# martinambrus/PitchExtractor

Measured on AMD Instinct MI355X. Metric: mel-frames/sec training throughput (JDCNet, 24 kHz, batch=256), higher is better.
Workload: dtype f32

## Files before the change

### pitchextractor_amd/csrc/act16.h

```cpp
#pragma once
#include "common.h"

namespace pe {

typedef __bf16 act16_t;

__device__ __forceinline__ float4 ld4(const float* p) { return *reinterpret_cast<const float4*>(p); }
__device__ __forceinline__ void st4(float* p, const float4& v) { *reinterpret_cast<float4*>(p) = v; }
__device__ __forceinline__ float ld1(const float* p) { return *p; }
__device__ __forceinline__ void st1(float* p, float v) { *p = v; }

__device__ __forceinline__ float4 ld4(const act16_t* p) {
  const uint2 u = *reinterpret_cast<const uint2*>(p);
  return make_float4(__uint_as_float(u.x << 16), __uint_as_float(u.x & 0xffff0000u), __uint_as_float(u.y << 16),
                     __uint_as_float(u.y & 0xffff0000u));
}
__device__ __forceinline__ unsigned pack_bf16_rne(float a, float b) {
  typedef __bf16 b2 __attribute__((ext_vector_type(2)));
  typedef float f2 __attribute__((ext_vector_type(2)));
  const f2 v = {a, b};
  return __builtin_bit_cast(unsigned, __builtin_convertvector(v, b2));
}
__device__ __forceinline__ void st4(act16_t* p, const float4& v) {
  *reinterpret_cast<uint2*>(p) = make_uint2(pack_bf16_rne(v.x, v.y), pack_bf16_rne(v.z, v.w));
}
__device__ __forceinline__ float ld1(const act16_t* p) {
  return __uint_as_float((unsigned)*reinterpret_cast<const unsigned short*>(p) << 16);
}
__device__ __forceinline__ void st1(act16_t* p, float v) { *p = (act16_t)v; }

template <class T> struct RawQuad;
template <> struct RawQuad<float> { typedef float4 type; };
template <> struct RawQuad<act16_t> { typedef uint2 type; };
__device__ __forceinline__ float4 ldraw(const float* p) { return *reinterpret_cast<const float4*>(p); }
__device__ __forceinline__ uint2 ldraw(const act16_t* p) { return *reinterpret_cast<const uint2*>(p); }
__device__ __forceinline__ float4 widen(const float4& v) { return v; }
__device__ __forceinline__ float4 widen(const uint2& u) {
  return make_float4(__uint_as_float(u.x << 16), __uint_as_float(u.x & 0xffff0000u), __uint_as_float(u.y << 16),
                     __uint_as_float(u.y & 0xffff0000u));
}
template <class T> __device__ __forceinline__ typename RawQuad<T>::type ldraw_buffer(__amdgpu_buffer_rsrc_t rs, unsigned voff, unsigned soff);
template <> __device__ __forceinline__ float4 ldraw_buffer<float>(__amdgpu_buffer_rsrc_t rs, unsigned voff, unsigned soff) {
  typedef unsigned int u4 __attribute__((ext_vector_type(4)));
  const u4 d = __builtin_amdgcn_raw_buffer_load_b128(rs, voff, soff, 0);
  return make_float4(__uint_as_float(d.x), __uint_as_float(d.y), __uint_as_float(d.z), __uint_as_float(d.w));
}
template <> __device__ __forceinline__ uint2 ldraw_buffer<act16_t>(__amdgpu_buffer_rsrc_t rs, unsigned voff, unsigned soff) {
  typedef unsigned int u2 __attribute__((ext_vector_type(2)));
  const u2 d = __builtin_amdgcn_raw_buffer_load_b64(rs, voff, soff, 0);
  return make_uint2(d.x, d.y);
}
template <class R> __device__ __forceinline__ R zero_raw();
template <> __device__ __forceinline__ float4 zero_raw<float4>() { return make_float4(0.f, 0.f, 0.f, 0.f); }
template <> __device__ __forceinline__ uint2 zero_raw<uint2>() { return make_uint2(0u, 0u); }

}
```

### pitchextractor_amd/csrc/common.h

```cpp
#pragma once
#include <hip/hip_runtime.h>
#include <stdint.h>
#include "../../include/pitchextractor_hip.h"

#define PE_CHECK_HIP(expr)                              \
  do {                                                  \
    hipError_t _e = (expr);                             \
    if (_e != hipSuccess) return (int)_e;               \
  } while (0)

#define PE_LAUNCH_CHECK()                               \
  do {                                                  \
    hipError_t _e = hipGetLastError();                  \
    if (_e != hipSuccess) return (int)_e;               \
  } while (0)

static inline hipStream_t pe_stream(void* s) { return reinterpret_cast<hipStream_t>(s); }

static inline int pe_unserved(int products) {
  return products >= PE_PROD_NATIVE && products <= PE_PROD_F16 ? PE_E_UNSUPPORTED : PE_E_ARG;
}

static inline int pe_cdiv(long a, long b) { return (int)((a + b - 1) / b); }

typedef float f32x4 __attribute__((ext_vector_type(4)));
typedef float f32x16 __attribute__((ext_vector_type(16)));

#define PE_WAVE 64

__device__ __forceinline__ double pe_wave_strided_sum(const double* base, long stride, int n) {
  const int lane = threadIdx.x & 63;
  double s = 0.0;
  for (int z = lane; z < n; z += 64) s += base[(long)z * stride];
#pragma unroll
  for (int off = 32; off > 0; off >>= 1) s += __shfl_down(s, off, 64);
  return s;
}

static inline int pe_pick_splits(int tiles, long K, int min_k_per_split, int resident) {
  long max_s = K / min_k_per_split;
  if (max_s < 1) max_s = 1;
  if (max_s > 1024) max_s = 1024;
  int best = 1;
  double best_score = -1.0;
  for (int sp = 1; sp <= (int)max_s; ++sp) {
    const long wgs = (long)tiles * sp;
    const long waves = (wgs + resident - 1) / resident;
    const double eff = (double)wgs / (double)(waves * resident);
    const double score = eff - 0.0001 * sp + (wgs >= 2L * resident ? 0.05 : 0.0);
    if (score > best_score) { best_score = score; best = sp; }
  }
  return best;
}

__device__ __forceinline__ float4 pe_ordered_slab_sum4(const float* __restrict__ ws, long slab_stride, int splits,
                                                       long i4) {
  const float4* p = reinterpret_cast<const float4*>(ws) + i4;
  const long st4 = slab_stride >> 2;
  double sx = 0.0, sy = 0.0, sz = 0.0, sw = 0.0;
  int z = 0;
  for (; z + 8 <= splits; z += 8) {
    float4 v[8];
#pragma unroll
    for (int u = 0; u < 8; ++u) v[u] = p[(long)(z + u) * st4];
#pragma unroll
    for (int u = 0; u < 8; ++u) { sx += (double)v[u].x; sy += (double)v[u].y; sz += (double)v[u].z; sw += (double)v[u].w; }
  }
  for (; z < splits; ++z) {
    const float4 v = p[(long)z * st4];
    sx += (double)v.x; sy += (double)v.y; sz += (double)v.z; sw += (double)v.w;
  }
  return make_float4((float)sx, (float)sy, (float)sz, (float)sw);
}

__device__ __forceinline__ void philox_round(uint32_t (&c)[4], uint32_t (&k)[2]) {
  const uint32_t M0 = 0xD2511F53u, M1 = 0xCD9E8D57u;
  const uint64_t p0 = (uint64_t)M0 * c[0], p1 = (uint64_t)M1 * c[2];
  const uint32_t n0 = (uint32_t)(p1 >> 32) ^ c[1] ^ k[0];
  const uint32_t n1 = (uint32_t)p1;
  const uint32_t n2 = (uint32_t)(p0 >> 32) ^ c[3] ^ k[1];
  const uint32_t n3 = (uint32_t)p0;
  c[0] = n0; c[1] = n1; c[2] = n2; c[3] = n3;
  k[0] += 0x9E3779B9u; k[1] += 0xBB67AE85u;
}

__device__ __forceinline__ void philox4(uint64_t seed, uint64_t ctr, uint32_t (&out)[4]) {
  uint32_t c[4] = {(uint32_t)ctr, (uint32_t)(ctr >> 32), 0u, 0u};
  uint32_t k[2] = {(uint32_t)seed, (uint32_t)(seed >> 32)};
#pragma unroll
  for (int i = 0; i < 10; ++i) philox_round(c, k);
  out[0] = c[0]; out[1] = c[1]; out[2] = c[2]; out[3] = c[3];
}

__device__ __forceinline__ bool pe_dropout_keep(uint32_t word, float p) {
  return ((float)(word >> 8) * (1.0f / 16777216.0f)) >= p;
}
```

### pitchextractor_amd/csrc/conv.hip

```cpp
#include <type_traits>
#include "forms.h"

namespace {
using namespace pe;
typedef unsigned int u32x4_t __attribute__((ext_vector_type(4)));
typedef unsigned int u32x2_t __attribute__((ext_vector_type(2)));

__global__ void repack3x3_kernel(const float* __restrict__ w, float* __restrict__ w_fwd,
                                 float* __restrict__ w_dgrad, int Cout, int Cin) {
  const int idx = blockIdx.x * blockDim.x + threadIdx.x;
  if (idx >= Cout * Cin * 9) return;
  const int tap = idx % 9, ci = (idx / 9) % Cin, co = idx / (9 * Cin);
  const float v = w[idx];
  if (w_fwd) w_fwd[((long)co * 9 + tap) * Cin + ci] = v;
  if (w_dgrad) w_dgrad[((long)ci * 9 + (8 - tap)) * Cout + co] = v;
}

__global__ void transpose2d_kernel(const float* __restrict__ in, float* __restrict__ out, int rows, int cols) {
  __shared__ float tile[32][33];
  const int c0 = blockIdx.x * 32, r0 = blockIdx.y * 32;
  for (int i = threadIdx.y; i < 32; i += 8) {
    const int r = r0 + i, c = c0 + threadIdx.x;
    tile[i][threadIdx.x] = (r < rows && c < cols) ? in[(long)r * cols + c] : 0.f;
  }
  __syncthreads();
  for (int i = threadIdx.y; i < 32; i += 8) {
    const int c = c0 + i, r = r0 + threadIdx.x;
    if (r < rows && c < cols) out[(long)c * rows + r] = tile[threadIdx.x][i];
  }
}

template <class TO>
struct ConvEpiT {
  TO* Y;
  int rows, N, accumulate;
  double* stats;
  __device__ __forceinline__ void operator()(int row, int col, float v) const {
    if (row < rows && col < N) {
      TO* d = Y + (long)row * N + col;
      if (accumulate) v += ld1(d);
      st1(d, v);
    }
  }
};
typedef ConvEpiT<float> ConvEpi;

template <class TO> __device__ __forceinline__ float stored_value(float v) {
  if constexpr (std::is_same<TO, float>::value) return v;
  else return __uint_as_float(pack_bf16_rne(v, 0.f) << 16);
}

template <class TL, int MODE, class TA = float, class TH = __bf16>
__global__ __launch_bounds__(256) void conv3x3_kernel(ConvLoader<TL::A_LOADS, TA> al, RowLoader bl, ConvEpiT<TA> ep,
                                                      int K, int tiles_m, int tiles_n, const unsigned* amax_x,
                                                      const unsigned* amax_w) {
  __shared__ __attribute__((aligned(16))) float As[TL::BM * nt_row_floats<MODE>()];
  __shared__ __attribute__((aligned(16))) float Bs[TL::BN * nt_row_floats<MODE>()];
  const int tile = xcd_remap(blockIdx.x, tiles_m * tiles_n);
  const int m0 = (tile / tiles_n) * TL::BM, n0 = (tile % tiles_n) * TL::BN;
  al.init(m0);
  bl.init(n0);
  f32x16 acc[TL::TM][TL::TN];
  zero_acc<TL>(acc);
  H2Scales hs{1.f, 1.f, 1.f};
  if constexpr (MODE == kSplit2) hs.load(amax_x, amax_w);
  nt_mainloop_mode<TL, MODE, false, 1, TH>(al, bl, K, As, Bs, acc, hs.sa, hs.sb);
  for_each_acc<TL>(acc, [&](int r, int c, float v) { ep(m0 + r, n0 + c, MODE == kSplit2 ? hs.unscale(v) : v); });
}

template <class TL, class FM, class TA = typename FM::TA>
int launch_conv(const TA* x, const float* wp, TA* y, int B, int T, int F, int C, int N, int accumulate,
                hipStream_t st, const unsigned* amax_x, const unsigned* amax_w) {
  const int rows = B * T * F, K = 9 * C;
  ConvLoader<TL::A_LOADS, TA> al;
  al.p = x; al.T = T; al.F = F; al.C = C; al.rows = rows;
  RowLoader bl{wp, (long)K, N, K, 0};
  ConvEpiT<TA> ep{y, rows, N, accumulate, nullptr};
  const int tm = pe_cdiv(rows, TL::BM), tn = pe_cdiv(N, TL::BN);
  hipLaunchKernelGGL((conv3x3_kernel<TL, FM::MODE, TA, typename FM::TH>), dim3(tm * tn), dim3(256), 0, st, al, bl, ep, K,
                     tm, tn, amax_x, amax_w);
  PE_LAUNCH_CHECK();
  return PE_OK;
}


template <int NT, class TH = __bf16>
__global__ void wfrag_pack_kernel(const float* __restrict__ w, long ld, int N, int K, uint4* __restrict__ out,
                                  const unsigned* __restrict__ amax = nullptr) {
  const long idx = (long)blockIdx.x * blockDim.x + threadIdx.x;
  const int NB32 = (N + 31) >> 5, KB = K >> 4;
  const int lane = (int)(idx & 63);
  const long blk = idx >> 6;
  if (blk >= (long)NB32 * KB) return;
  const int nb = (int)(blk % NB32), kb = (int)(blk / NB32);
  const int n = nb * 32 + (lane & 31), k = kb * 16 + (lane >> 5) * 8;
  float4 v0 = make_float4(0.f, 0.f, 0.f, 0.f), v1 = v0;
  if (n < N) {
    v0 = *reinterpret_cast<const float4*>(w + (long)n * ld + k);
    v1 = *reinterpret_cast<const float4*>(w + (long)n * ld + k + 4);
  }
  uint4* dst = out + ((long)(kb * NB32 + nb) * NT) * 64 + lane;
  if constexpr (NT == 3) {
    const Split3 a = split3(v0), b = split3(v1);
    dst[0] = make_uint4(a.hi.x, a.hi.y, b.hi.x, b.hi.y);
    dst[64] = make_uint4(a.mid.x, a.mid.y, b.mid.x, b.mid.y);
    dst[128] = make_uint4(a.lo.x, a.lo.y, b.lo.x, b.lo.y);
  } else if constexpr (NT == 2) {
    const float sc = h2_scale(*amax);
    const Split2 a = split2(v0, sc), b = split2(v1, sc);
    dst[0] = make_uint4(a.hi.x, a.hi.y, b.hi.x, b.hi.y);
    dst[64] = make_uint4(a.lo.x, a.lo.y, b.lo.x, b.lo.y);
  } else {
    const half4<TH> a = to_half4<TH>(v0), b = to_half4<TH>(v1);
    const uint2 ua = __builtin_bit_cast(uint2, a), ub = __builtin_bit_cast(uint2, b);
    dst[0] = make_uint4(ua.x, ua.y, ub.x, ub.y);
  }
}

template <int BN, int MODE, int PASSES, int D, bool FA2, class TA = float, class TH = __bf16>
__global__ __launch_bounds__(256, 2) void conv3x3_halo_wf_kernel(const TA* __restrict__ x,
                                                                 const uint4* __restrict__ wf, ConvEpiT<TA> ep, int T,
                                                                 int F, int C, int N, int P, int tiles_m,
                                                                 int tiles_n, const unsigned* amax_x,
                                                                 const unsigned* amax_w) {
  constexpr int NT = mode_terms<MODE>();
  using H = term_t<NT, TH>;
  H2Scales hs{1.f, 1.f, 1.f};
  if constexpr (MODE == kSplit2) hs.load(amax_x, amax_w);
  constexpr int TM = 2, TN = BN / 64, WN = BN / 2;
  constexpr int ZR = PASSES * 32;
  constexpr int AIMG = (ZR + 4) * 32;
  constexpr int S = 18 * TN;
  static_assert(S % D == 0 && D >= 2, "the fragment ring wraps at chunk boundaries");
  __shared__ __attribute__((aligned(16))) H As[NT * AIMG];
  const int tid = threadIdx.x, lane = tid & 63, wv = tid >> 6;
  const int wm = wv >> 1, wn = wv & 1, r = lane & 31, h = lane >> 5;
  const int tile = xcd_remap(blockIdx.x, tiles_m * tiles_n);
  const int p0 = (tile / tiles_n) * 128, n0 = (tile % tiles_n) * BN;
  const int WR = 128 + 2 * F + 2;
  const int srow = tid >> 3, piece = tid & 7;
  const int nchunks = C / 32;

  unsigned vbits[TM];
#pragma unroll
  for (int i = 0; i < TM; ++i) {
    const int p = p0 + wm * 64 + i * 32 + r;
    unsigned b = 0;
    if (p < P) {
      const int f = p % F, t = (p / F) % T;
#pragma unroll
      for (int tap = 0; tap < 9; ++tap) {
        const int tt = t + tap / 3 - 1, ff = f + tap % 3 - 1;
        if (tt >= 0 && tt < T && ff >= 0 && ff < F) b |= 1u << tap;
      }
    }
    vbits[i] = b;
  }

  typedef typename RawQuad<TA>::type Raw;
  Raw ra[PASSES];
  const __amdgpu_buffer_rsrc_t xrs = __builtin_amdgcn_make_buffer_rsrc(
      const_cast<TA*>(x), 0, (unsigned)((long)P * C * (long)sizeof(TA)), 0x00020000);
  unsigned voa[PASSES];
#pragma unroll
  for (int ps = 0; ps < PASSES; ++ps) {
    const int wr = ps * 32 + srow;
    const long q = (long)p0 - F - 1 + wr;
    voa[ps] = (wr < WR && q >= 0 && q < P) ? (unsigned)((q * C + piece * 4) * (long)sizeof(TA)) : 0x80000000u;
  }
  auto fetch_a = [&](int cc) {
    const unsigned so = (unsigned)(cc * 32 * (int)sizeof(TA));
#pragma unroll
    for (int ps = 0; ps < PASSES; ++ps) {
      if constexpr (std::is_same<TA, float>::value) {
        const u32x4_t d = __builtin_amdgcn_raw_buffer_load_b128(xrs, voa[ps], so, 0);
        ra[ps] = make_float4(__uint_as_float(d.x), __uint_as_float(d.y), __uint_as_float(d.z), __uint_as_float(d.w));
      } else {
        const u32x2_t d = __builtin_amdgcn_raw_buffer_load_b64(xrs, voa[ps], so, 0);
        ra[ps] = make_uint2(d.x, d.y);
      }
    }
  };

  const int NB32 = (N + 31) >> 5, kb_tap = C >> 4;
  const int kb_stride = NB32 * NT * 64;
  const __amdgpu_buffer_rsrc_t wrs = __builtin_amdgcn_make_buffer_rsrc(
      const_cast<uint4*>(wf), 0, (unsigned)((long)9 * kb_tap * kb_stride * 16), 0x00020000);
  unsigned vow[TN];
#pragma unroll
  for (int j = 0; j < TN; ++j) {
    const int nb = (n0 + wn * WN + j * 32) >> 5;
    vow[j] = (unsigned)(((nb < NB32 ? nb : NB32 - 1) * NT * 64 + lane) * 16);
  }
  half8<H> ring[D][NT];
  auto issue = [&](int slot, int cc, int s) {
    const int j = s % TN, kk = (s / TN) & 1, tap = s / (2 * TN);
    const unsigned so = (unsigned)((tap * kb_tap + cc * 2 + kk) * kb_stride) * 16u;
#pragma unroll
    for (int c = 0; c < NT; ++c)
      ring[slot][c] = __builtin_bit_cast(half8<H>, __builtin_amdgcn_raw_buffer_load_b128(wrs, vow[j], so + (unsigned)c * 1024u, 0));
  };

  f32x16 acc[TM][TN];
#pragma unroll
  for (int i = 0; i < TM; ++i)
#pragma unroll
    for (int j = 0; j < TN; ++j)
#pragma unroll
      for (int g = 0; g < 16; ++g) acc[i][j][g] = 0.f;

  if (tid < 8) {
#pragma unroll
    for (int c = 0; c < NT; ++c) *reinterpret_cast<uint2*>(As + c * AIMG + ZR * 32 + tid * 4) = make_uint2(0u, 0u);
  }
  fetch_a(0);
#pragma unroll
  for (int s = 0; s < D - 1; ++s) issue(s, 0, s);

  auto load_fa = [&](half8<H> (&fa)[TM][NT], int tap, int kk) {
    const int shift = (tap / 3) * F + tap % 3;
#pragma unroll
    for (int i = 0; i < TM; ++i) {
      const int row = (vbits[i] >> tap) & 1u ? wm * 64 + i * 32 + r + shift : ZR;
#pragma unroll
      for (int c = 0; c < NT; ++c)
        fa[i][c] = *reinterpret_cast<const half8<H>*>(As + c * AIMG + swz_off(row, kk * 2 + h));
    }
  };

  for (int cc = 0; cc < nchunks; ++cc) {
    __syncthreads();
#pragma unroll
    for (int ps = 0; ps < PASSES; ++ps) halo_store<NT>(As, AIMG, ps * 32 + srow, piece, ra[ps], hs.sa);
    __syncthreads();
    if (cc + 1 < nchunks) fetch_a(cc + 1);
    half8<H> fa[FA2 ? 2 : 1][TM][NT];
    if (FA2) load_fa(fa[0], 0, 0);
#pragma unroll
    for (int s = 0; s < S; ++s) {
      const int j = s % TN, blk = s / TN;
      {
        const int sn = s + D - 1;
        if (sn < S) issue(sn % D, cc, sn);
        else if (cc + 1 < nchunks) issue(sn % D, cc + 1, sn - S);
      }
      if (FA2) {
        if (j == 0 && blk + 1 < 18) load_fa(fa[(blk + 1) & 1], (blk + 1) >> 1, (blk + 1) & 1);
      } else if (j == 0) {
        load_fa(fa[0], blk >> 1, blk & 1);
      }
      const int fs = FA2 ? (blk & 1) : 0;
#pragma unroll
      for (int i = 0; i < TM; ++i) acc[i][j] = mfma_terms<NT>(fa[fs][i], ring[s % D], acc[i][j]);
      __builtin_amdgcn_sched_barrier(0);
    }
  }
  double s1[TN], s2[TN];
#pragma unroll
  for (int j = 0; j < TN; ++j) s1[j] = s2[j] = 0.0;
#pragma unroll
  for (int i = 0; i < TM; ++i)
#pragma unroll
    for (int j = 0; j < TN; ++j)
#pragma unroll
      for (int g = 0; g < 16; ++g) {
        const int row = p0 + wm * 64 + i * 32 + (g & 3) + 8 * (g >> 2) + 4 * h, col = n0 + wn * WN + j * 32 + r;
        if (row < ep.rows && col < ep.N) {
          TA* d = ep.Y + (long)row * ep.N + col;
          float v = MODE == kSplit2 ? hs.unscale(acc[i][j][g]) : acc[i][j][g];
          if (ep.accumulate) v += ld1(d);
          st1(d, v);
          v = stored_value<TA>(v);
          s1[j] += (double)v;
          s2[j] += (double)v * (double)v;
        }
      }
  if (ep.stats) {
#pragma unroll
    for (int j = 0; j < TN; ++j) {
      s1[j] += __shfl_xor(s1[j], 32, 64);
      s2[j] += __shfl_xor(s2[j], 32, 64);
    }
    __syncthreads();
    double* red = reinterpret_cast<double*>(As);
    if (h == 0) {
#pragma unroll
      for (int j = 0; j < TN; ++j) {
        red[(wm * BN + wn * WN + j * 32 + r) * 2] = s1[j];
        red[(wm * BN + wn * WN + j * 32 + r) * 2 + 1] = s2[j];
      }
    }
    __syncthreads();
    const long tile_m = tile / tiles_n;
    for (int c = tid; c < BN; c += 256) {
      if (n0 + c < ep.N) {
        ep.stats[(tile_m * 2) * ep.N + n0 + c] = red[c * 2] + red[(BN + c) * 2];
        ep.stats[(tile_m * 2 + 1) * ep.N + n0 + c] = red[c * 2 + 1] + red[(BN + c) * 2 + 1];
      }
    }
  }
}

template <int BN, class FM, int PASSES, int D, bool FA2, class TA = typename FM::TA>
int launch_conv_halo_wf(const TA* x, const void* wf, TA* y, int B, int T, int F, int C, int N, int accumulate,
                        double* stats, hipStream_t st, const unsigned* amax_x, const unsigned* amax_w) {
  const int P = B * T * F;
  ConvEpiT<TA> ep{y, P, N, accumulate, stats};
  const int tm = pe_cdiv(P, 128), tn = pe_cdiv(N, BN);
  hipLaunchKernelGGL((conv3x3_halo_wf_kernel<BN, FM::MODE, PASSES, D, FA2, TA, typename FM::TH>), dim3(tm * tn),
                     dim3(256), 0, st, x, reinterpret_cast<const uint4*>(wf), ep, T, F, C, N, P, tm, tn, amax_x, amax_w);
  PE_LAUNCH_CHECK();
  return PE_OK;
}

static inline size_t pe_wfrag_bytes_host(int N, int K, int terms) { return (size_t)((N + 31) / 32) * (K / 16) * terms * 1024; }

int conv_halo_passes(int F, int N) {
  const int wr = 128 + 2 * F + 2;
  if (wr <= 7 * 32 && N >= 96) return 7;
  if (wr <= 10 * 32 && N <= 64) return 10;
  return 0;
}

template <int BM, int BN>
__global__ __launch_bounds__(256) void conv3x3_wgrad_kernel(const float* __restrict__ dy, const float* __restrict__ x,
                                                            float* __restrict__ ws, int T, int F, int Cin,
                                                            int Cout, int P, int k_per_split, int tiles_n,
                                                            int n_tiles, int n_chunks) {
  __shared__ __attribute__((aligned(16))) float As[kBK * BM];
  __shared__ __attribute__((aligned(16))) float Bs[kBK * BN];
  const int xcd = blockIdx.x & 7, q = blockIdx.x >> 3;
  const int tap = q % 9;
  const int chunk = (q / 9) * 8 + xcd;
  if (chunk >= n_chunks) return;
  const int tile = chunk % n_tiles, split = chunk / n_tiles;
  const int m0 = (tile / tiles_n) * BM, n0 = (tile % tiles_n) * BN;
  const int kb = split * k_per_split;
  const int ke = min(P, kb + k_per_split);
  KRowLoader<BM> al{dy, (long)Cout, Cout, 0};
  ShiftedPixelLoader<BN> bl;
  bl.p = x; bl.T = T; bl.F = F; bl.C = Cin; bl.dt = tap / 3 - 1; bl.df = tap % 3 - 1;
  al.init(m0, kb);
  bl.init(n0, kb);
  f32x16 acc[BM / 64][BN / 64];
#pragma unroll
  for (int i = 0; i < BM / 64; ++i)
#pragma unroll
    for (int j = 0; j < BN / 64; ++j)
#pragma unroll
      for (int g = 0; g < 16; ++g) acc[i][j][g] = 0.f;
  tn_mainloop<BM, BN>(al, bl, kb, ke, As, Bs, acc);
  float* dst = ws + ((long)split * 9 + tap) * Cout * Cin;
  tn_for_each_acc<BM, BN>(acc, [&](int r, int c, float v) {
    const int co = m0 + r, ci = n0 + c;
    if (co < Cout && ci < Cin) dst[(long)co * Cin + ci] = v;
  });
}

template <int DUMMY>
__global__ __launch_bounds__(256, 2) void conv3x3_wgrad9_kernel(const float* __restrict__ dy,
                                                                const float* __restrict__ x,
                                                                float* __restrict__ ws, int T, int F, int Cin,
                                                                int Cout, int P, int k_per_split, int tiles_n) {
  __shared__ __attribute__((aligned(16))) float Ys[kBK * 64];
  __shared__ __attribute__((aligned(16))) float Xs[3 * 34 * 64];
  __shared__ float Mk[3 * 34 * 4];
  const int tid = threadIdx.x, lane = tid & 63, wv = tid >> 6;
  const int wm = wv >> 1, wn = wv & 1, r = lane & 31, h = lane >> 5;
  const int tiles_mn = (Cout / 64) * tiles_n;
  const int lin = xcd_remap(blockIdx.x, gridDim.x);
  const int tile_id = lin % tiles_mn, split_id = lin / tiles_mn;
  const int m0 = (tile_id / tiles_n) * 64, n0 = (tile_id % tiles_n) * 64;
  const int kb = split_id * k_per_split;
  const int ke = min(P, kb + k_per_split);

  f32x16 acc[9];
#pragma unroll
  for (int tp = 0; tp < 9; ++tp)
#pragma unroll
    for (int q = 0; q < 16; ++q) acc[tp][q] = 0.f;

  const int c4 = (tid & 15) * 4;
  float4 ry[2], rx[7];
  auto fetch = [&](int k0) {
#pragma unroll
    for (int i = 0; i < 2; ++i) {
      const int k = k0 + (tid >> 4) + 16 * i;
      ry[i] = k < ke ? *reinterpret_cast<const float4*>(dy + (long)k * Cout + m0 + c4)
                     : make_float4(0.f, 0.f, 0.f, 0.f);
    }
#pragma unroll
    for (int i = 0; i < 7; ++i) {
      const int wr = (tid >> 4) + 16 * i;
      rx[i] = make_float4(0.f, 0.f, 0.f, 0.f);
      if (wr < 102) {
        const int w = wr / 34, row = wr - w * 34;
        const long q = (long)k0 + (long)(w - 1) * F + row - 1;
        if (q >= 0 && q < P) rx[i] = *reinterpret_cast<const float4*>(x + q * Cin + n0 + c4);
      }
    }
  };
  fetch(kb);
  for (int k0 = kb; k0 < ke; k0 += kBK) {
    __syncthreads();
#pragma unroll
    for (int i = 0; i < 2; ++i) *reinterpret_cast<float4*>(Ys + ((tid >> 4) + 16 * i) * 64 + c4) = ry[i];
#pragma unroll
    for (int i = 0; i < 7; ++i) {
      const int wr = (tid >> 4) + 16 * i;
      if (wr < 102) *reinterpret_cast<float4*>(Xs + wr * 64 + c4) = rx[i];
    }
    if (tid < 102) {
      const int w = tid / 34, row = tid - w * 34;
      const long q = (long)k0 + (long)(w - 1) * F + row - 1;
      float m0v = 0.f, m1v = 0.f, m2v = 0.f;
      if (q >= 0 && q < P) {
        const int fq = (int)(q % F), tq = (int)((q / F) % T);
        const bool trow = !((w == 2 && tq == 0) || (w == 0 && tq == T - 1));
        m0v = (trow && fq != F - 1) ? 1.f : 0.f;
        m1v = trow ? 1.f : 0.f;
        m2v = (trow && fq != 0) ? 1.f : 0.f;
      }
      Mk[tid * 4 + 0] = m0v; Mk[tid * 4 + 1] = m1v; Mk[tid * 4 + 2] = m2v;
    }
    __syncthreads();
    if (k0 + kBK < ke) fetch(k0 + kBK);
    const float* a_rd = Ys + wm * 32 + r;
    const float* b_rd = Xs + wn * 32 + r;
#pragma unroll 4
    for (int s = 0; s < kBK / 2; ++s) {
      const int k = 2 * s + h;
      const float a = a_rd[k * 64];
#pragma unroll
      for (int w = 0; w < 3; ++w)
#pragma unroll
        for (int d = 0; d < 3; ++d) {
          const int row = k + d;
          const float b = b_rd[(w * 34 + row) * 64] * Mk[(w * 34 + row) * 4 + d];
          acc[w * 3 + d] = mfma32(a, b, acc[w * 3 + d]);
        }
    }
  }
#pragma unroll
  for (int tp = 0; tp < 9; ++tp) {
    float* dst = ws + ((long)split_id * 9 + tp) * Cout * Cin;
#pragma unroll
    for (int q = 0; q < 16; ++q) {
      const int co = m0 + wm * 32 + (q & 3) + 8 * (q >> 2) + 4 * h;
      const int ci = n0 + wn * 32 + r;
      dst[(long)co * Cin + ci] = acc[tp][q];
    }
  }
}

template <int NT, bool HALO, class TA = float, class TH = __bf16>
__global__ __launch_bounds__(256, 2) void conv3x3_wgrad9_x3_kernel(const TA* __restrict__ dy,
                                                                   const TA* __restrict__ x,
                                                                   float* __restrict__ ws, int T, int F, int Cin,
                                                                   int Cout, int P, int k_per_split, int tiles_n,
                                                                   const unsigned* amax_dy, const unsigned* amax_x) {
// ... 549 lines not shown
```

### pitchextractor_amd/csrc/gemm.hip

```cpp
#include <stdlib.h>
#include <type_traits>
#include <utility>
#include "forms.h"


namespace {
using namespace pe;
typedef unsigned int u32x4 __attribute__((ext_vector_type(4)));

bool aligned16(const void* p) { return (reinterpret_cast<uintptr_t>(p) & 15) == 0; }

template <class TO>
struct StoreEpiT {
  TO* C;
  long ldc;
  const float* bias0;
  const float* bias1;
  int M, N, accumulate;
  __device__ __forceinline__ void operator()(int row, int col, float v) const {
    if (row < M && col < N) {
      if (bias0) v += bias0[col];
      if (bias1) v += bias1[col];
      TO* dst = C + (long)row * ldc + col;
      if (accumulate) v += ld1(dst);
      st1(dst, v);
    }
  }
};
typedef StoreEpiT<float> StoreEpi;

template <class TL, int MODE, class TA = float, class TH = __bf16>
__global__ __launch_bounds__(256) void gemm_nt_kernel(RowLoaderT<TA> al, RowLoader bl, StoreEpiT<TA> ep, int K,
                                                      int tiles_m, int tiles_n, const unsigned* amax_a,
                                                      const unsigned* amax_b) {
  __shared__ __attribute__((aligned(16))) float As[TL::BM * nt_row_floats<MODE>()];
  __shared__ __attribute__((aligned(16))) float Bs[TL::BN * nt_row_floats<MODE>()];
  const int tile = xcd_remap(blockIdx.x, tiles_m * tiles_n);
  const int m0 = (tile / tiles_n) * TL::BM, n0 = (tile % tiles_n) * TL::BN;
  al.init(m0);
  bl.init(n0);
  f32x16 acc[TL::TM][TL::TN];
  zero_acc<TL>(acc);
  H2Scales hs{1.f, 1.f, 1.f};
  if constexpr (MODE == kSplit2) hs.load(amax_a, amax_b);
  nt_mainloop_mode<TL, MODE, false, 1, TH>(al, bl, K, As, Bs, acc, hs.sa, hs.sb);
  for_each_acc<TL>(acc, [&](int r, int c, float v) { ep(m0 + r, n0 + c, MODE == kSplit2 ? hs.unscale(v) : v); });
}

template <class TL, int MODE, class TA = float, class TH = __bf16>
__global__ __launch_bounds__(256, ((MODE == kSplit || MODE == kSplit2) && TL::BM == 128 && TL::BN == 128) ? 3 : 1)
void gemm_nt_t_kernel(RowLoaderT<TA> al, RowLoader bl, StoreEpiT<TA> ep, int K, int tiles_m, int tiles_n,
                      const unsigned* amax_a, const unsigned* amax_b) {
  using TT = Tile<TL::BN, TL::BM, TL::WAVES_N, TL::WAVES_M>;
  __shared__ __attribute__((aligned(16))) float As[TL::BM * nt_row_floats<MODE>()];
  __shared__ __attribute__((aligned(16))) float Bs[TL::BN * nt_row_floats<MODE>()];
  const int tile = xcd_remap(blockIdx.x, tiles_m * tiles_n);
  const int m0 = (tile / tiles_n) * TL::BM, n0 = (tile % tiles_n) * TL::BN;
  al.init(m0);
  bl.init(n0);
  f32x16 acc[TT::TM][TT::TN];
  zero_acc<TT>(acc);
  H2Scales hs{1.f, 1.f, 1.f};
  if constexpr (MODE == kSplit2) hs.load(amax_a, amax_b);
  nt_mainloop_mode<TT, MODE, true, 1, TH>(bl, al, K, Bs, As, acc, hs.sb, hs.sa);
  const int lane = threadIdx.x & 63, wv = threadIdx.x >> 6;
  const int wn = wv / TT::WAVES_N, wm = wv % TT::WAVES_N;
  const int r = lane & 31, h = lane >> 5;
#pragma unroll
  for (int i = 0; i < TT::TM; ++i)
#pragma unroll
    for (int q = 0; q < 4; ++q) {
      const int col = n0 + wn * TT::WM + i * 32 + 8 * q + 4 * h;
      if (col >= ep.N) continue;
      float4 b0 = make_float4(0.f, 0.f, 0.f, 0.f), b1 = b0;
      if (ep.bias0) b0 = make_float4(ep.bias0[col], ep.bias0[col + 1], ep.bias0[col + 2], ep.bias0[col + 3]);
      if (ep.bias1) b1 = make_float4(ep.bias1[col], ep.bias1[col + 1], ep.bias1[col + 2], ep.bias1[col + 3]);
#pragma unroll
      for (int j = 0; j < TT::TN; ++j) {
        const int row = m0 + wm * TT::WN + j * 32 + r;
        if (row >= ep.M) continue;
        TA* dst = ep.C + (long)row * ep.ldc + col;
        float4 v = make_float4(acc[i][j][4 * q], acc[i][j][4 * q + 1], acc[i][j][4 * q + 2], acc[i][j][4 * q + 3]);
        if constexpr (MODE == kSplit2) {
          v.x = hs.unscale(v.x); v.y = hs.unscale(v.y); v.z = hs.unscale(v.z); v.w = hs.unscale(v.w);
        }
        if (ep.bias0) { v.x += b0.x; v.y += b0.y; v.z += b0.z; v.w += b0.w; }
        if (ep.bias1) { v.x += b1.x; v.y += b1.y; v.z += b1.z; v.w += b1.w; }
        if (ep.accumulate) { const float4 o = ld4(dst); v.x += o.x; v.y += o.y; v.z += o.z; v.w += o.w; }
        st4(dst, v);
      }
    }
}

template <class TL, class F, class TA = typename F::TA>
int launch_nt(const RowLoaderT<TA>& al, const RowLoader& bl, const StoreEpiT<TA>& ep, int M, int N, int K,
              hipStream_t st, const unsigned* amax_a, const unsigned* amax_b) {
  constexpr int MODE = F::MODE;
  using TH = typename F::TH;
  const int tm = pe_cdiv(M, TL::BM), tn = pe_cdiv(N, TL::BN);
  const bool vec = MODE != kNative && (N & 3) == 0 && (ep.ldc & 3) == 0 &&
                   (reinterpret_cast<uintptr_t>(ep.C) & (4 * sizeof(TA) - 1)) == 0;
  if (vec)
    hipLaunchKernelGGL((gemm_nt_t_kernel<TL, MODE, TA, TH>), dim3(tm * tn), dim3(256), 0, st, al, bl, ep, K, tm, tn,
                       amax_a, amax_b);
  else
    hipLaunchKernelGGL((gemm_nt_kernel<TL, MODE, TA, TH>), dim3(tm * tn), dim3(256), 0, st, al, bl, ep, K, tm, tn, amax_a,
                       amax_b);
  PE_LAUNCH_CHECK();
  return PE_OK;
}

template <int BM, int BN, int MODE, class TA = float, class TH = __bf16>
__global__ __launch_bounds__(256) void gemm_tn_kernel(KRowLoader<BM, TA> al, KRowLoader<BN, TA> bl, float* out,
                                                      long ldo, long split_stride, int M, int N, int K,
                                                      int k_per_split, int tiles_n, int accumulate,
                                                      const unsigned* amax_a, const unsigned* amax_b) {
  __shared__ __attribute__((aligned(16))) float As[tn_lds_floats<MODE, BM>()];
  __shared__ __attribute__((aligned(16))) float Bs[tn_lds_floats<MODE, BN>()];
  const int tiles_mn = ((M + BM - 1) / BM) * tiles_n;
  const int lin = xcd_remap(blockIdx.x, gridDim.x);
  const int tile_id = lin % tiles_mn, split_id = lin / tiles_mn;
  const int m0 = (tile_id / tiles_n) * BM, n0 = (tile_id % tiles_n) * BN;
  const int kb = split_id * k_per_split;
  const int ke = min(K, kb + k_per_split);
  al.init(m0, kb);
  bl.init(n0, kb);
  f32x16 acc[BM / 64][BN / 64];
#pragma unroll
  for (int i = 0; i < BM / 64; ++i)
#pragma unroll
    for (int j = 0; j < BN / 64; ++j)
#pragma unroll
      for (int g = 0; g < 16; ++g) acc[i][j][g] = 0.f;
  H2Scales hs{1.f, 1.f, 1.f};
  if constexpr (MODE == kSplit2) hs.load(amax_a, amax_b);
  tn_mainloop_mode<MODE, BM, BN, 1, TH>(al, bl, kb, ke, As, Bs, acc, hs.sa, hs.sb);
  float* dst = out + (long)split_id * split_stride;
  tn_for_each_acc<BM, BN>(acc, [&](int r, int c, float v) {
    const int row = m0 + r, col = n0 + c;
    if constexpr (MODE == kSplit2) v = hs.unscale(v);
    if (row < M && col < N) {
      float* d = dst + (long)row * ldo + col;
      if (accumulate) v += *d;
      *d = v;
    }
  });
}

__global__ void splitk_reduce_kernel(const float* ws, long split_stride, int splits, float* C, long ldc,
                                     int M, int N, int accumulate) {
  const long i4 = (long)blockIdx.x * blockDim.x + threadIdx.x;
  if (i4 * 4 >= (long)M * N) return;
  const float4 s = pe_ordered_slab_sum4(ws, split_stride, splits, i4);
  const long idx = i4 * 4;
  const int row = (int)(idx / N), col = (int)(idx - (long)row * N);
  float* d = C + (long)row * ldc + col;
  if (accumulate) { d[0] += s.x; d[1] += s.y; d[2] += s.z; d[3] += s.w; }
  else { d[0] = s.x; d[1] = s.y; d[2] = s.z; d[3] = s.w; }
}

void tn_plan(int M, int N, int K, int bm, int bn, int mode, int* splits, int* k_per_split) {
  const int tiles = pe_cdiv(M, bm) * pe_cdiv(N, bn);
  const int s = pe_pick_splits(tiles, K, 512, (mode == kSplit || mode == kSplit2) ? 512 : 768);
  int kps = pe_cdiv(K, s);
  kps = (kps + kBK - 1) / kBK * kBK;
  *splits = pe_cdiv(K, kps);
  *k_per_split = kps;
}

template <int BM, int BN, class F, class TA = typename F::TA>
int launch_tn(const TA* A, long lda, const TA* B, long ldb, float* C, long ldc, int M, int N, int K,
              int accumulate, float* ws, size_t ws_bytes, hipStream_t st, const unsigned* amax_a,
              const unsigned* amax_b) {
  constexpr int MODE = F::MODE;
  using TH = typename F::TH;
  int splits, kps;
  tn_plan(M, N, K, BM, BN, MODE, &splits, &kps);
  KRowLoader<BM, TA> al{A, lda, M, 0};
  KRowLoader<BN, TA> bl{B, ldb, N, 0};
  const int tm = pe_cdiv(M, BM), tn = pe_cdiv(N, BN);
  if (splits == 1) {
    hipLaunchKernelGGL((gemm_tn_kernel<BM, BN, MODE, TA, TH>), dim3(tm * tn, 1), dim3(256), 0, st, al, bl, C, ldc, 0L, M, N,
                       K, kps, tn, accumulate, amax_a, amax_b);
    PE_LAUNCH_CHECK();
    return PE_OK;
  }
  const size_t need = (size_t)splits * M * N * sizeof(float);
  if (!ws || ws_bytes < need) return PE_E_WORKSPACE;
  hipLaunchKernelGGL((gemm_tn_kernel<BM, BN, MODE, TA, TH>), dim3(tm * tn * splits), dim3(256), 0, st, al, bl, ws, (long)N,
                     (long)M * N, M, N, K, kps, tn, 0, amax_a, amax_b);
  PE_LAUNCH_CHECK();
  const long total = (long)M * N;
  hipLaunchKernelGGL(splitk_reduce_kernel, dim3(pe_cdiv(total / 4, 256)), dim3(256), 0, st, ws, (long)M * N, splits,
                     C, ldc, M, N, accumulate);
  PE_LAUNCH_CHECK();
  return PE_OK;
}

}

template <class F, class TA = typename F::TA>
static int gemm_nt_impl(const TA* A, long lda, const float* B, long ldb, TA* C, long ldc, int M, int N,
                        int K, const float* bias0, const float* bias1, int accumulate, void* stream,
                        const unsigned* amax_a, const unsigned* amax_b) {
  constexpr int MODE = F::MODE;
  if (!A || !B || !C || M < 0 || N < 0 || K <= 0) return PE_E_ARG;
  if (MODE == kSplit2 && (!amax_a || !amax_b)) return PE_E_ARG;
  if (M == 0 || N == 0) return PE_OK;
  if ((K & 3) || (lda & 3) || (ldb & 3) || (reinterpret_cast<uintptr_t>(A) & (4 * sizeof(TA) - 1)) || !aligned16(B))
    return PE_E_UNSUPPORTED;
  if (lda < 0 || ldb < 0 || lda >= (1L << 21) || ldb >= (1L << 21)) return PE_E_UNSUPPORTED;
  RowLoaderT<TA> al{A, lda, M, K, 0};
  RowLoader bl{B, ldb, N, K, 0};
  StoreEpiT<TA> ep{C, ldc, bias0, bias1, M, N, accumulate};
  hipStream_t st = pe_stream(stream);
  if (N <= 32) return launch_nt<Tile<128, 32, 4, 1>, F>(al, bl, ep, M, N, K, st, amax_a, amax_b);
  if (N <= 64) return launch_nt<Tile<256, 64, 4, 1>, F>(al, bl, ep, M, N, K, st, amax_a, amax_b);
  if (N % 192 == 0 && (N % 128 != 0 || MODE != kNative))
    return launch_nt<Tile<128, 192, 2, 2>, F>(al, bl, ep, M, N, K, st, amax_a, amax_b);
  return launch_nt<Tile<128, 128, 2, 2>, F>(al, bl, ep, M, N, K, st, amax_a, amax_b);
}

extern "C" int pe_gemm_nt(int products, int act16, const void* A, long lda, const float* B, long ldb, void* C, long ldc,
                          int M, int N, int K, const float* bias0, const float* bias1, int accumulate,
                          const unsigned* amax_a, const unsigned* amax_b, void* stream) {
  return with_form<kAllForms, true>(products, act16, [&](auto f) {
    using TA = typename decltype(f)::TA;
    return gemm_nt_impl<decltype(f)>(static_cast<const TA*>(A), lda, B, ldb, static_cast<TA*>(C), ldc, M, N, K, bias0,
                                     bias1, accumulate, stream, amax_a, amax_b);
  });
}

extern "C" size_t pe_gemm_tn_workspace_bytes(int M, int N, int K) {
  if (M <= 0 || N <= 0 || K <= 0) return 0;
  size_t need = 0;
  for (int mode : {kNative, kSplit}) {
    int splits, kps;
    tn_plan(M, N, K, M <= 64 ? 64 : 128, N <= 64 ? 64 : 128, mode, &splits, &kps);
    const size_t b = splits > 1 ? (size_t)splits * M * N * sizeof(float) : 0;
    need = b > need ? b : need;
  }
  return need;
}

template <class F, class TA = typename F::TA>
static int gemm_tn_impl(const TA* A, long lda, const TA* B, long ldb, float* C, long ldc, int M, int N,
                        int K, int accumulate, float* workspace, size_t workspace_bytes, void* stream,
                        const unsigned* amax_a, const unsigned* amax_b) {
  constexpr int MODE = F::MODE;
  if (!A || !B || !C || M < 0 || N < 0 || K <= 0) return PE_E_ARG;
  if (MODE == kSplit2 && (!amax_a || !amax_b)) return PE_E_ARG;
  if (M == 0 || N == 0) return PE_OK;
  if ((M & 3) || (N & 3) || (lda & 3) || (ldb & 3) || (reinterpret_cast<uintptr_t>(A) & (4 * sizeof(TA) - 1)) ||
      (reinterpret_cast<uintptr_t>(B) & (4 * sizeof(TA) - 1)))
    return PE_E_UNSUPPORTED;
  if (lda < 0 || ldb < 0 || lda >= (1L << 24) || ldb >= (1L << 24)) return PE_E_UNSUPPORTED;
  hipStream_t st = pe_stream(stream);
// ... 23 lines not shown
```

Before: 615,100.

## Use buffer loads/stores with bounds-check masking in GEMM and conv epilogues

Rewrites the conv3x3 and NT-GEMM epilogues to use AMD raw buffer stores and loads. Out-of-range rows and columns are discarded by the hardware bounds check instead of per-element branches, and accumulate reads and bias reads are prefetched one group ahead, separated by sched barriers. The NT kernel's launch-bounds occupancy rule also changes. This aims to cut branch and address arithmetic in the epilogue and hide the latency of the read-modify-write, at the cost of more registers and a 2 GB size limit; an environment variable falls back to the old pointer path.

```diff
diff --git a/pitchextractor_amd/csrc/act16.h b/pitchextractor_amd/csrc/act16.h
--- a/pitchextractor_amd/csrc/act16.h
+++ b/pitchextractor_amd/csrc/act16.h
@@ -50,6 +50,32 @@
   const u2 d = __builtin_amdgcn_raw_buffer_load_b64(rs, voff, soff, 0);
   return make_uint2(d.x, d.y);
 }
+__device__ __forceinline__ unsigned ld1raw_buffer(const float*, __amdgpu_buffer_rsrc_t rs, unsigned voff) {
+  return __builtin_amdgcn_raw_buffer_load_b32(rs, voff, 0, 0);
+}
+__device__ __forceinline__ unsigned ld1raw_buffer(const act16_t*, __amdgpu_buffer_rsrc_t rs, unsigned voff) {
+  return (unsigned)(unsigned short)__builtin_amdgcn_raw_buffer_load_b16(rs, voff, 0, 0);
+}
+__device__ __forceinline__ float widen1(const float*, unsigned raw) { return __uint_as_float(raw); }
+__device__ __forceinline__ float widen1(const act16_t*, unsigned raw) { return __uint_as_float(raw << 16); }
+__device__ __forceinline__ void st1_buffer(float*, __amdgpu_buffer_rsrc_t rs, unsigned voff, float v) {
+  __builtin_amdgcn_raw_buffer_store_b32(__float_as_uint(v), rs, voff, 0, 0);
+}
+__device__ __forceinline__ void st1_buffer(act16_t*, __amdgpu_buffer_rsrc_t rs, unsigned voff, float v) {
+  __builtin_amdgcn_raw_buffer_store_b16(__builtin_bit_cast(unsigned short, (act16_t)v), rs, voff, 0, 0);
+}
+__device__ __forceinline__ void st4_buffer(float*, __amdgpu_buffer_rsrc_t rs, unsigned voff, const float4& v) {
+  typedef unsigned int u4 __attribute__((ext_vector_type(4)));
+  const u4 d = {__float_as_uint(v.x), __float_as_uint(v.y), __float_as_uint(v.z), __float_as_uint(v.w)};
+  __builtin_amdgcn_raw_buffer_store_b128(d, rs, voff, 0, 0);
+}
+__device__ __forceinline__ void st4_buffer(act16_t*, __amdgpu_buffer_rsrc_t rs, unsigned voff, const float4& v) {
+  typedef unsigned int u2 __attribute__((ext_vector_type(2)));
+  const u2 d = {pack_bf16_rne(v.x, v.y), pack_bf16_rne(v.z, v.w)};
+  __builtin_amdgcn_raw_buffer_store_b64(d, rs, voff, 0, 0);
+}
+constexpr unsigned kBufferOutside = 0x80000000u;
+
 template <class R> __device__ __forceinline__ R zero_raw();
 template <> __device__ __forceinline__ float4 zero_raw<float4>() { return make_float4(0.f, 0.f, 0.f, 0.f); }
 template <> __device__ __forceinline__ uint2 zero_raw<uint2>() { return make_uint2(0u, 0u); }
diff --git a/pitchextractor_amd/csrc/common.h b/pitchextractor_amd/csrc/common.h
--- a/pitchextractor_amd/csrc/common.h
+++ b/pitchextractor_amd/csrc/common.h
@@ -1,6 +1,8 @@
 #pragma once
 #include <hip/hip_runtime.h>
 #include <stdint.h>
+#include <stdlib.h>
+#include <string.h>
 #include "../../include/pitchextractor_hip.h"
 
 #define PE_CHECK_HIP(expr)                              \
@@ -22,6 +24,14 @@
 }
 
 static inline int pe_cdiv(long a, long b) { return (int)((a + b - 1) / b); }
+
+static inline int pe_epilogue_buffer(long out_bytes) {
+  static const int forced_pointer = [] {
+    const char* e = getenv("PE_EPILOGUE");
+    return e && strcmp(e, "pointer") == 0 ? 1 : 0;
+  }();
+  return !forced_pointer && out_bytes < (1L << 31);
+}
 
 typedef float f32x4 __attribute__((ext_vector_type(4)));
 typedef float f32x16 __attribute__((ext_vector_type(16)));
diff --git a/pitchextractor_amd/csrc/conv.hip b/pitchextractor_amd/csrc/conv.hip
--- a/pitchextractor_amd/csrc/conv.hip
+++ b/pitchextractor_amd/csrc/conv.hip
@@ -35,6 +35,7 @@
   TO* Y;
   int rows, N, accumulate;
   double* stats;
+  int buffer;
   __device__ __forceinline__ void operator()(int row, int col, float v) const {
     if (row < rows && col < N) {
       TO* d = Y + (long)row * N + col;
@@ -258,23 +259,72 @@
   double s1[TN], s2[TN];
 #pragma unroll
   for (int j = 0; j < TN; ++j) s1[j] = s2[j] = 0.0;
-#pragma unroll
-  for (int i = 0; i < TM; ++i)
-#pragma unroll
-    for (int j = 0; j < TN; ++j)
+  const int row0 = p0 + wm * 64 + 4 * h;
+  auto add_stat = [&](int j, int row, float v) {
+    v = __uint_as_float(__float_as_uint(stored_value<TA>(v)) & (row < ep.rows ? 0xffffffffu : 0u));
+    s1[j] += (double)v;
+    s2[j] += (double)v * (double)v;
+  };
+  const bool stats = ep.stats != nullptr;
+  auto epilogue_buffer = [&](auto acc_tag) {
+    constexpr bool ACC = decltype(acc_tag)::value;
+    const __amdgpu_buffer_rsrc_t yrs = __builtin_amdgcn_make_buffer_rsrc(
+        ep.Y, 0, (unsigned)((long)ep.rows * ep.N * (long)sizeof(TA)), 0x00020000);
+    const unsigned rowb = (unsigned)ep.N * (unsigned)sizeof(TA);
+    unsigned vo[TN];
+#pragma unroll
+    for (int j = 0; j < TN; ++j) {
+      const int col = n0 + wn * WN + j * 32 + r;
+      vo[j] = col < ep.N ? (unsigned)row0 * rowb + (unsigned)col * (unsigned)sizeof(TA) : kBufferOutside;
+    }
+    auto voff = [&](int i, int j, int g) { return vo[j] + (unsigned)(i * 32 + (g & 3) + 8 * (g >> 2)) * rowb; };
+    unsigned old[2][16];
+    auto fetch_old = [&](int b) {
+#pragma unroll
+      for (int g = 0; g < 16; ++g) old[b & 1][g] = ld1raw_buffer(ep.Y, yrs, voff(b / TN, b % TN, g));
+    };
+    if constexpr (ACC) fetch_old(0);
+#pragma unroll
+    for (int b = 0; b < TM * TN; ++b) {
+      const int i = b / TN, j = b % TN;
+      if constexpr (ACC) {
+        if (b + 1 < TM * TN) fetch_old(b + 1);
+        __builtin_amdgcn_sched_barrier(0);
+      }
+      float v[16];
 #pragma unroll
       for (int g = 0; g < 16; ++g) {
-        const int row = p0 + wm * 64 + i * 32 + (g & 3) + 8 * (g >> 2) + 4 * h, col = n0 + wn * WN + j * 32 + r;
-        if (row < ep.rows && col < ep.N) {
-          TA* d = ep.Y + (long)row * ep.N + col;
-          float v = MODE == kSplit2 ? hs.unscale(acc[i][j][g]) : acc[i][j][g];
-          if (ep.accumulate) v += ld1(d);
-          st1(d, v);
-          v = stored_value<TA>(v);
-          s1[j] += (double)v;
-          s2[j] += (double)v * (double)v;
+        v[g] = MODE == kSplit2 ? hs.unscale(acc[i][j][g]) : acc[i][j][g];
+        if constexpr (ACC) v[g] += widen1(ep.Y, old[b & 1][g]);
+        st1_buffer(ep.Y, yrs, voff(i, j, g), v[g]);
+      }
+      if (stats) {
+#pragma unroll
+        for (int g = 0; g < 16; ++g) add_stat(j, row0 + i * 32 + (g & 3) + 8 * (g >> 2), v[g]);
+      }
+      if constexpr (ACC) __builtin_amdgcn_sched_barrier(0);
+    }
+  };
+  auto epilogue_pointer = [&]() {
+#pragma unroll
+    for (int i = 0; i < TM; ++i)
+#pragma unroll
+      for (int j = 0; j < TN; ++j)
+#pragma unroll
+        for (int g = 0; g < 16; ++g) {
+          const int row = row0 + i * 32 + (g & 3) + 8 * (g >> 2), col = n0 + wn * WN + j * 32 + r;
+          if (row < ep.rows && col < ep.N) {
+            TA* d = ep.Y + (long)row * ep.N + col;
+            float v = MODE == kSplit2 ? hs.unscale(acc[i][j][g]) : acc[i][j][g];
+            if (ep.accumulate) v += ld1(d);
+            st1(d, v);
+            if (stats) add_stat(j, row, v);
+          }
         }
-      }
+  };
+  if (!ep.buffer) epilogue_pointer();
+  else if (ep.accumulate) epilogue_buffer(std::true_type{});
+  else epilogue_buffer(std::false_type{});
   if (ep.stats) {
 #pragma unroll
     for (int j = 0; j < TN; ++j) {
@@ -305,7 +355,7 @@
 int launch_conv_halo_wf(const TA* x, const void* wf, TA* y, int B, int T, int F, int C, int N, int accumulate,
                         double* stats, hipStream_t st, const unsigned* amax_x, const unsigned* amax_w) {
   const int P = B * T * F;
-  ConvEpiT<TA> ep{y, P, N, accumulate, stats};
+  ConvEpiT<TA> ep{y, P, N, accumulate, stats, pe_epilogue_buffer((long)(P + 128) * N * (long)sizeof(TA))};
   const int tm = pe_cdiv(P, 128), tn = pe_cdiv(N, BN);
   hipLaunchKernelGGL((conv3x3_halo_wf_kernel<BN, FM::MODE, PASSES, D, FA2, TA, typename FM::TH>), dim3(tm * tn),
                      dim3(256), 0, st, x, reinterpret_cast<const uint4*>(wf), ep, T, F, C, N, P, tm, tn, amax_x, amax_w);
diff --git a/pitchextractor_amd/csrc/gemm.hip b/pitchextractor_amd/csrc/gemm.hip
--- a/pitchextractor_amd/csrc/gemm.hip
+++ b/pitchextractor_amd/csrc/gemm.hip
@@ -47,8 +47,11 @@
   for_each_acc<TL>(acc, [&](int r, int c, float v) { ep(m0 + r, n0 + c, MODE == kSplit2 ? hs.unscale(v) : v); });
 }
 
-template <class TL, int MODE, class TA = float, class TH = __bf16>
-__global__ __launch_bounds__(256, ((MODE == kSplit || MODE == kSplit2) && TL::BM == 128 && TL::BN == 128) ? 3 : 1)
+template <class TL, int MODE> constexpr int nt_t_min_blocks() {
+  return TL::BM * TL::BN == 128 * 128 && !(MODE == kSplit && TL::BM == 256) ? 3 : 1;
+}
+template <class TL, int MODE, bool BUF, class TA = float, class TH = __bf16>
+__global__ __launch_bounds__(256, (nt_t_min_blocks<TL, MODE>()))
 void gemm_nt_t_kernel(RowLoaderT<TA> al, RowLoader bl, StoreEpiT<TA> ep, int K, int tiles_m, int tiles_n,
                       const unsigned* amax_a, const unsigned* amax_b) {
   using TT = Tile<TL::BN, TL::BM, TL::WAVES_N, TL::WAVES_M>;
@@ -66,30 +69,87 @@
   const int lane = threadIdx.x & 63, wv = threadIdx.x >> 6;
   const int wn = wv / TT::WAVES_N, wm = wv % TT::WAVES_N;
   const int r = lane & 31, h = lane >> 5;
-#pragma unroll
-  for (int i = 0; i < TT::TM; ++i)
-#pragma unroll
-    for (int q = 0; q < 4; ++q) {
-      const int col = n0 + wn * TT::WM + i * 32 + 8 * q + 4 * h;
-      if (col >= ep.N) continue;
-      float4 b0 = make_float4(0.f, 0.f, 0.f, 0.f), b1 = b0;
-      if (ep.bias0) b0 = make_float4(ep.bias0[col], ep.bias0[col + 1], ep.bias0[col + 2], ep.bias0[col + 3]);
-      if (ep.bias1) b1 = make_float4(ep.bias1[col], ep.bias1[col + 1], ep.bias1[col + 2], ep.bias1[col + 3]);
-#pragma unroll
-      for (int j = 0; j < TT::TN; ++j) {
-        const int row = m0 + wm * TT::WN + j * 32 + r;
-        if (row >= ep.M) continue;
-        TA* dst = ep.C + (long)row * ep.ldc + col;
-        float4 v = make_float4(acc[i][j][4 * q], acc[i][j][4 * q + 1], acc[i][j][4 * q + 2], acc[i][j][4 * q + 3]);
-        if constexpr (MODE == kSplit2) {
-          v.x = hs.unscale(v.x); v.y = hs.unscale(v.y); v.z = hs.unscale(v.z); v.w = hs.unscale(v.w);
+  auto quad = [&](int i, int q, int j) {
+    float4 v = make_float4(acc[i][j][4 * q], acc[i][j][4 * q + 1], acc[i][j][4 * q + 2], acc[i][j][4 * q + 3]);
+    if constexpr (MODE == kSplit2) {
+      v.x = hs.unscale(v.x); v.y = hs.unscale(v.y); v.z = hs.unscale(v.z); v.w = hs.unscale(v.w);
+    }
+    return v;
+  };
+  auto add4 = [](float4& v, const float4& o) { v.x += o.x; v.y += o.y; v.z += o.z; v.w += o.w; };
+  if constexpr (BUF) {
+    typedef typename RawQuad<TA>::type Raw;
+    const unsigned esz = (unsigned)sizeof(TA), rowb = (unsigned)ep.ldc * esz;
+    const __amdgpu_buffer_rsrc_t crs = __builtin_amdgcn_make_buffer_rsrc(
+        ep.C, 0, (unsigned)(((long)(ep.M - 1) * ep.ldc + ep.N) * (long)sizeof(TA)), 0x00020000);
+    const unsigned nbytes = (unsigned)ep.N * 4u;
+    const __amdgpu_buffer_rsrc_t b0rs = __builtin_amdgcn_make_buffer_rsrc(const_cast<float*>(ep.bias0), 0, ep.bias0 ? nbytes : 0u, 0x00020000);
+    const __amdgpu_buffer_rsrc_t b1rs = __builtin_amdgcn_make_buffer_rsrc(const_cast<float*>(ep.bias1), 0, ep.bias1 ? nbytes : 0u, 0x00020000);
+    const unsigned rowo = (unsigned)(m0 + wm * TT::WN + r) * rowb;
+    constexpr int G = TT::TM * 4;
+    auto col_of = [&](int g) { return n0 + wn * TT::WM + (g >> 2) * 32 + 8 * (g & 3) + 4 * h; };
+    auto voff = [&](int g, int j) {
+      const int col = col_of(g);
+      return (col < ep.N ? rowo + (unsigned)col * esz : kBufferOutside) + (unsigned)(j * 32) * rowb;
+    };
+    const float4 nz = make_float4(-0.f, -0.f, -0.f, -0.f);
+    const bool has0 = ep.bias0 != nullptr, has1 = ep.bias1 != nullptr;
+    auto run = [&](auto acc_tag) {
+      constexpr bool ACC = decltype(acc_tag)::value;
+      Raw old[2][TT::TN];
+      float4 b0[2], b1[2];
+      auto fetch = [&](int g) {
+        const int col = col_of(g);
+        const unsigned bo = col < ep.N ? (unsigned)col * 4u : kBufferOutside;
+        b0[g & 1] = ldraw_buffer<float>(b0rs, bo, 0u);
+        b1[g & 1] = ldraw_buffer<float>(b1rs, bo, 0u);
+        if constexpr (ACC) {
+#pragma unroll
+          for (int j = 0; j < TT::TN; ++j) old[g & 1][j] = ldraw_buffer<TA>(crs, voff(g, j), 0u);
         }
-        if (ep.bias0) { v.x += b0.x; v.y += b0.y; v.z += b0.z; v.w += b0.w; }
-        if (ep.bias1) { v.x += b1.x; v.y += b1.y; v.z += b1.z; v.w += b1.w; }
-        if (ep.accumulate) { const float4 o = ld4(dst); v.x += o.x; v.y += o.y; v.z += o.z; v.w += o.w; }
-        st4(dst, v);
+      };
+      fetch(0);
+#pragma unroll
+      for (int g = 0; g < G; ++g) {
+        if (g + 1 < G) fetch(g + 1);
+        __builtin_amdgcn_sched_barrier(0);
+        const float4 c0 = has0 ? b0[g & 1] : nz, c1 = has1 ? b1[g & 1] : nz;
+#pragma unroll
+        for (int j = 0; j < TT::TN; ++j) {
+          float4 v = quad(g >> 2, g & 3, j);
+          add4(v, c0);
+          add4(v, c1);
+          if constexpr (ACC) add4(v, widen(old[g & 1][j]));
+          st4_buffer(ep.C, crs, voff(g, j), v);
+        }
+        __builtin_amdgcn_sched_barrier(0);
       }
-    }
+    };
+    if (ep.accumulate) run(std::true_type{});
+    else run(std::false_type{});
+  } else {
+#pragma unroll
+    for (int i = 0; i < TT::TM; ++i)
+#pragma unroll
+      for (int q = 0; q < 4; ++q) {
+        const int col = n0 + wn * TT::WM + i * 32 + 8 * q + 4 * h;
+        if (col >= ep.N) continue;
+        float4 b0 = make_float4(0.f, 0.f, 0.f, 0.f), b1 = b0;
+        if (ep.bias0) b0 = make_float4(ep.bias0[col], ep.bias0[col + 1], ep.bias0[col + 2], ep.bias0[col + 3]);
+        if (ep.bias1) b1 = make_float4(ep.bias1[col], ep.bias1[col + 1], ep.bias1[col + 2], ep.bias1[col + 3]);
+#pragma unroll
+        for (int j = 0; j < TT::TN; ++j) {
+          const int row = m0 + wm * TT::WN + j * 32 + r;
+          if (row >= ep.M) continue;
+          TA* dst = ep.C + (long)row * ep.ldc + col;
+          float4 v = quad(i, q, j);
+          if (ep.bias0) add4(v, b0);
+          if (ep.bias1) add4(v, b1);
+          if (ep.accumulate) add4(v, ld4(dst));
+          st4(dst, v);
+        }
+      }
+  }
 }
 
 template <class TL, class F, class TA = typename F::TA>
@@ -100,9 +160,14 @@
   const int tm = pe_cdiv(M, TL::BM), tn = pe_cdiv(N, TL::BN);
   const bool vec = MODE != kNative && (N & 3) == 0 && (ep.ldc & 3) == 0 &&
                    (reinterpret_cast<uintptr_t>(ep.C) & (4 * sizeof(TA) - 1)) == 0;
-  if (vec)
-    hipLaunchKernelGGL((gemm_nt_t_kernel<TL, MODE, TA, TH>), dim3(tm * tn), dim3(256), 0, st, al, bl, ep, K, tm, tn,
-                       amax_a, amax_b);
+  if (vec) {
+    if (ep.ldc >= N && pe_epilogue_buffer((long)(M + TL::BM) * ep.ldc * (long)sizeof(TA)))
+      hipLaunchKernelGGL((gemm_nt_t_kernel<TL, MODE, true, TA, TH>), dim3(tm * tn), dim3(256), 0, st, al, bl, ep, K, tm,
+                         tn, amax_a, amax_b);
+    else
+      hipLaunchKernelGGL((gemm_nt_t_kernel<TL, MODE, false, TA, TH>), dim3(tm * tn), dim3(256), 0, st, al, bl, ep, K, tm,
+                         tn, amax_a, amax_b);
+  }
   else
     hipLaunchKernelGGL((gemm_nt_kernel<TL, MODE, TA, TH>), dim3(tm * tn), dim3(256), 0, st, al, bl, ep, K, tm, tn, amax_a,
                        amax_b);
```

After: 636,100, median of 6. 3.4% higher.
